# bmds-lab/Crackling

Measured on AMD Instinct MI355X. Metric: guides/sec (whole node) + achieved HBM GB/s, 20bp/<=4mm ISSL scan, higher is better.
Workload: dtype u32

## Files before the change

crackling_amd/csrc/issl_bin.hip:

```cpp
#include <hip/hip_runtime.h>

#include <algorithm>
#include <type_traits>

#include "issl_kernels.hpp"

namespace issl {


__global__ __launch_bounds__(256) void k_pack_scan_stream(ImageView v, uint32_t *__restrict__ scan_out,
                                                          uint64_t *__restrict__ esig_out,
                                                          uint8_t *__restrict__ occ8_out,
                                                          uint32_t *__restrict__ error_flag, uint32_t *__restrict__ seen,
                                                          uint32_t tile_begin, uint32_t tile_end)
{
    for (uint32_t t = tile_begin + blockIdx.x; t < tile_end; t += gridDim.x) {
        uint32_t lo = 0, hi = v.n_buckets;
        while (hi - lo > 1) {
            const uint32_t mid = (lo + hi) >> 1;
            if (v.tile_first[mid] <= t) lo = mid; else hi = mid;
        }
        const uint32_t b = lo;
        const uint32_t slice = b >> v.slice_width;
        const uint64_t start = v.bucket_start[b];
// ... 533 lines not shown
        }
        __syncthreads();
        const uint32_t n_here = total - i0 < THREADS ? total - i0 : THREADS;
        const uint4 *src4 = reinterpret_cast<const uint4 *>(l.stage);
        uint4 *dst4 = reinterpret_cast<uint4 *>(fitems + base.items + i0);
        for (uint32_t q = w; q < n_here * 3u; q += THREADS) dst4[q] = src4[q];
        __syncthreads();
    }
}

template <uint32_t WAYS, uint32_t THREADS>
__device__ __forceinline__ void fine_scatter_guides(const ImageView &v, uint32_t b, const uint32_t *__restrict__ gstart,
                                                    const uint32_t *__restrict__ gfill, const uint32_t *__restrict__ gword,
                                                    const uint32_t *__restrict__ gidx, const uint64_t *__restrict__ gsig,
                                                    const uint32_t *__restrict__ fcount, const uint32_t *__restrict__ fcount0,
                                                    const FineSum *__restrict__ fbase, uint32_t *__restrict__ fword,
                                                    FineMeta *__restrict__ fmeta, FineGuideLds<THREADS> &l)
{
    constexpr uint32_t ways = WAYS;
    const uint32_t w = threadIdx.x, slice = b >> v.slice_width;
    const uint32_t g0 = gstart[b], n = gfill[b];
    const uint32_t base_slots = fbase[b].slots;
    uint32_t c = 0, c1 = 0;
    if (w < 256u) {
        c = fcount[static_cast<uint64_t>(b) * 256u + w];
        c1 = c - fcount0[static_cast<uint64_t>(b) * 256u + w];
    }
    uint32_t i = w, guide = 0, word = 0;
    uint64_t sig = 0;
    if (i < n) { guide = gidx[g0 + i]; word = gword[g0 + i]; sig = gsig[g0 + i]; }
    const uint32_t slots = (c + kGuideGroup - 1u) / kGuideGroup * kGuideGroup;
    const uint32_t slot_at = base_slots + static_cast<uint32_t>(block_exclusive_scan(slots, l.scan, nullptr));
    if (w < 256u) {
        l.slot_of[w] = slot_at;
        l.slot0_of[w] = slot_at + c1;
        l.cursor[w] = 0;
        l.cursor0[w] = 0;
        l.has_cands[w] = c ? 1u : 0u;
        for (uint32_t k2 = c; k2 < slots; ++k2) { fmeta[slot_at + k2] = FineMeta{kNoGuide, 0u, 0ull}; fword[slot_at + k2] = kPadGuideWord; }
    }
    __syncthreads();
    while (i < n) {
        const uint32_t gj = succ_byte(sig, slice, v.slice_width);
        const uint32_t word12 = fine_word(word, slice, v.slice_width);
#pragma unroll
        for (uint32_t way = 0; way < ways; ++way) {
            const uint32_t ww = fine_way(gj, way);
            if (!l.has_cands[ww]) continue;
            const uint32_t slot = way ? l.slot_of[ww] + atomicAdd(&l.cursor[ww], 1u) : l.slot0_of[ww] + atomicAdd(&l.cursor0[ww], 1u);
            fword[slot] = word12 | (fine_class(way) << 24);
            fmeta[slot] = FineMeta{guide, (b << 8) | ww, sig};
        }
        i += THREADS;
        if (i < n) { guide = gidx[g0 + i]; word = gword[g0 + i]; sig = gsig[g0 + i]; }
    }
}

template <uint32_t WAYS, uint32_t THREADS>
__global__ __launch_bounds__(THREADS) void k_fine_scatter(ImageView v, const uint32_t *__restrict__ gstart,
                                                          const uint32_t *__restrict__ gfill, const uint32_t *__restrict__ gword,
                                                          const uint32_t *__restrict__ gidx, const uint64_t *__restrict__ gsig,
                                                          const uint32_t *__restrict__ fcount, const uint32_t *__restrict__ fcount0,
                                                          const FineSum *__restrict__ fbase, const PlanInfo *__restrict__ plan,
                                                          uint32_t *__restrict__ fword, FineMeta *__restrict__ fmeta,
                                                          ScanItem *__restrict__ fitems, uint32_t item_guides, uint32_t tail_shapes)
{
    short_kernel_priority();
    if (!plan->fine) return;
    __shared__ union { FineItemLds<THREADS> items; FineGuideLds<THREADS> guides; } lds;
    const uint32_t nb = v.n_buckets;
    if (blockIdx.x < nb) fine_scatter_items(v, blockIdx.x, fcount, fcount0, fbase, fitems, item_guides, tail_shapes, lds.items);
    else fine_scatter_guides<WAYS, THREADS>(v, blockIdx.x - nb, gstart, gfill, gword, gidx, gsig, fcount, fcount0, fbase, fword, fmeta, lds.guides);
}

__global__ __launch_bounds__(256) void k_fine_ranges(const PlanInfo *__restrict__ plan, const ScanItem *__restrict__ fitems,
                                                     RangeStart *__restrict__ starts)
{
    short_kernel_priority();
    if (!plan->fine) return;
    const uint32_t n_ranges = plan->n_ranges;
    const uint32_t r = blockIdx.x * 4u + (threadIdx.x >> 6);
    if (r <= n_ranges && n_ranges != 0) {
        const RangeStart st = range_start_of<true>(fitems, plan->n_items, plan->total_cost, n_ranges, r);
        if ((threadIdx.x & 63u) == 0u) starts[r] = st;
    }
}

// ... 67 lines not shown
    }
    uint64_t t_units, t_cost, t_cand, t_ref, t_valid;
    uint32_t item_at = static_cast<uint32_t>(block512_exclusive_scan(units, lds, &t_units)) + units_before;
    uint64_t cost_at = block512_exclusive_scan(cost, lds, &t_cost) + cost_before;
    (void)block512_exclusive_scan(cand, lds, &t_cand);
    (void)block512_exclusive_scan(ref, lds, &t_ref);
    const uint32_t slot_at = (static_cast<uint32_t>(block512_exclusive_scan(valid, lds, &t_valid)) + valid_before) * kGuideGroup;
    const uint64_t t_slots = t_valid * kGuideGroup;
    const bool overflow = t_units > ws.cap_fitems || t_slots > ws.cap_fslots;
    if (mine && !overflow && my_s1 > my_s0) {
        const uint32_t way = my_way, s0 = my_s0, s1 = my_s1;
        const uint32_t word12 = fine_word(image_word(sig, sl, v.slice_width, sorted_layout != 0u), sl, v.slice_width);
        const uint32_t ww = fine_way(gj, way);
        const uint32_t c1 = way ? 1u : 0u;
        uint4 *fw = reinterpret_cast<uint4 *>(ws.fword + slot_at);
        fw[0] = make_uint4(word12 | (fine_class(way) << 24), kPadGuideWord, kPadGuideWord, kPadGuideWord);
        fw[1] = make_uint4(kPadGuideWord, kPadGuideWord, kPadGuideWord, kPadGuideWord);
        ws.fmeta[slot_at] = FineMeta{g, (b << 8) | ww, sig};
#pragma unroll
        for (uint32_t k2 = 1; k2 < kGuideGroup; ++k2) ws.fmeta[slot_at + k2] = FineMeta{kNoGuide, 0u, 0ull};
        const GroupUnits gu = group_units(s0, s1, tail_shapes);
        for (uint32_t u = 0; u < gu.units; ++u) {
            const bool full = u < gu.n_full;
            const uint32_t shape = full ? 32u : gu.shape, cap = 64u * shape;
            const uint32_t wstart = gu.s0a + u * kTileCands;
            const uint64_t after = blen - wstart;
            ScanItem it;
            it.bucket = (b << 8) | ww;
            it.g0 = slot_at;
            it.g1 = slot_at + 1u;
            it.n_tiles = 1;
            it.cost0 = cost_at;
            it.tile0 = item_at;
            it.last_cands = after < cap ? static_cast<uint32_t>(after) : cap;
            it.group_abs = tf * 64u + (wstart >> 5);
// ... 74 lines not shown
    hipLaunchKernelGGL(k_guide_scatter, dim3(blocks + range_blocks), dim3(256), 0, stream, d_guides, n, v.slice_width,
                       v.n_slices, (v.srec || v.sid) ? 1u : 0u, nb, ws.gstart, ws.gfill, ws.gword, ws.gidx, ws.gbucket, ws.gsig, blocks, ws.plan, ws.items,
                       ws.range_start);
    if (prune_mode) {
        const uint32_t ways = fine_ways_of(prune_mode);
        const uint32_t tail_shapes = prune_mode == 3 ? 0u : static_cast<uint32_t>(tn.tail_shapes);
        auto launch_fine = [&](auto ways_tag) {
            constexpr uint32_t W = decltype(ways_tag)::value;
            hipLaunchKernelGGL(k_fine_count<W>, dim3(nb), dim3(256), 0, stream, v, ws.gsig, ws.gstart, ws.gfill, ws.fcount,
                               ws.fcount0, ws.fsum, tn.item_guides, tail_shapes);
            hipLaunchKernelGGL(k_fine_plan, dim3(1), dim3(256), 0, stream, ws.fsum, nb, ws.fitems,
                               static_cast<uint32_t>(ws.cap_fitems), static_cast<uint32_t>(ws.cap_fslots), ws.plan, tn.scan_blocks,
                               prune_mode, tn.prune == 1 ? 1u : 0u, ws.sticky, ws.counters);
            if (static_cast<uint64_t>(n) * v.n_slices > 256ull * nb)
                hipLaunchKernelGGL((k_fine_scatter<W, 512u>), dim3(2u * nb), dim3(512), 0, stream, v, ws.gstart, ws.gfill, ws.gword, ws.gidx, ws.gsig,
                                   ws.fcount, ws.fcount0, ws.fsum, ws.plan, ws.fword, ws.fmeta, ws.fitems, tn.item_guides, tail_shapes);
            else
                hipLaunchKernelGGL((k_fine_scatter<W, 256u>), dim3(2u * nb), dim3(256), 0, stream, v, ws.gstart, ws.gfill, ws.gword, ws.gidx, ws.gsig,
                                   ws.fcount, ws.fcount0, ws.fsum, ws.plan, ws.fword, ws.fmeta, ws.fitems, tn.item_guides, tail_shapes);
        };
        if (ways == 1u) launch_fine(std::integral_constant<uint32_t, 1u>{});
        else if (ways == kFineWays) launch_fine(std::integral_constant<uint32_t, kFineWays>{});
        else launch_fine(std::integral_constant<uint32_t, kFineWays2>{});
        hipLaunchKernelGGL(k_fine_ranges, dim3((tn.scan_blocks + 1u + 3u) / 4u), dim3(256), 0, stream, ws.plan, ws.fitems, ws.range_start);
    }
}

}
```

crackling_amd/csrc/issl_device.hpp:

```cpp
#pragma once
#include <cstddef>
#include <cstdint>
#include <string>

#include "issl_host.hpp"

namespace issl {

constexpr uint64_t kImageMagic = 0x314C535349444D41ull;
constexpr uint32_t kImageVersion = 9;
constexpr uint32_t kTileCands = 2048;
constexpr uint32_t kHeaderBytes = 4096;

struct ImageHeader {
    uint64_t magic;
    uint32_t version;
    uint32_t kind;
    uint64_t n_sites, seq_len, n_lines, slice_width, n_slices, n_scores_file;
    uint64_t n_buckets;
    uint64_t n_scores_unique;
    uint64_t n_tiles;
    uint64_t tile_cands;
    uint64_t total_bytes;
    uint64_t off_bucket_start, off_tile_first, off_score_mask, off_score_val, off_sites, off_entries,
// ... 192 lines not shown
#if defined(__HIPCC__)
__host__ __device__
#endif
inline uint64_t slot_pad(uint32_t occ, uint32_t dist) { return static_cast<uint64_t>(occ) | (static_cast<uint64_t>(dist) << 32); }
constexpr uint32_t kFineWays = 13;
constexpr uint32_t kFineWays2 = 67;
constexpr uint32_t kFetchPairs = 8;
constexpr uint32_t kPruneMaxGuides = 1u << 20;
constexpr uint32_t kPruneMaxGuides2 = 1u << 18;
inline uint32_t prune_max_guides(uint32_t prune_mode, uint32_t n_slices)
{
    const uint32_t m = prune_mode == 3 ? kPruneMaxGuides2 : kPruneMaxGuides;
    return n_slices > 10 ? m >> 2 : n_slices > 5 ? m >> 1 : m;
}

struct alignas(16) FineMeta {
    uint32_t guide;
    uint32_t where;
    uint64_t gsig;
};

struct Workspace {
    uint32_t *ng = nullptr;
    uint32_t *gfill = nullptr;
    uint32_t *gstart = nullptr;
    uint32_t *gword = nullptr;
    uint32_t *gidx = nullptr;
    uint32_t *gbucket = nullptr;
    uint64_t *gsig = nullptr;
    ScanItem *items = nullptr;
    uint32_t *fword = nullptr;
    FineMeta *fmeta = nullptr;
    ScanItem *fitems = nullptr;
    uint32_t *fcount = nullptr;
    uint32_t *fcount0 = nullptr;
    FineSum *fsum = nullptr;
    size_t cap_fslots = 0, cap_fitems = 0;
    uint32_t fine_ways = 0;
    PlanInfo *plan = nullptr;
    RangeStart *range_start = nullptr;
    uint64_t *raw = nullptr;
    uint32_t *raw_used = nullptr;
    size_t cap_chunks = 0;
    Counters *counters = nullptr;
    unsigned long long *scan_span = nullptr;
    uint32_t span_slot = 0;
    uint64_t *scan_count = nullptr;
// ... 59 lines not shown
```

crackling_amd/csrc/issl_kernels.hip:

```cpp
#include <hip/hip_runtime.h>

#include "issl_kernels.hpp"

namespace issl {


struct alignas(4 * kGuideGroup) GuideGroup {
    uint32_t w[kGuideGroup];
};


__device__ __forceinline__ uint64_t raw_record(uint32_t gslot, uint32_t tile, uint32_t offset)
{
    return (static_cast<uint64_t>(gslot) << 37) | (static_cast<uint64_t>(tile) << 11) | offset;
}

struct RawWriter {
    uint64_t *chunk;
    uint32_t fill;
    uint32_t left;
    uint32_t reserve;
};

__device__ __forceinline__ void raw_retire(const RawWriter &w, uint32_t lane, const uint64_t *raw, uint32_t *raw_used)
// ... 57 lines not shown
                                                     uint32_t thr, uint32_t keep)
{
    uint32_t m[16];
#pragma unroll
    for (int q = 0; q < 4; ++q) {
        const uint4 lo = gm[q], hi = gm[4 + q];
        asm volatile("" ::: "memory");
        m[4 * q + 0] = (c[4 * q + 0] ^ lo.x) | (c[16 + 4 * q + 0] ^ hi.x);
        m[4 * q + 1] = (c[4 * q + 1] ^ lo.y) | (c[16 + 4 * q + 1] ^ hi.y);
        m[4 * q + 2] = (c[4 * q + 2] ^ lo.z) | (c[16 + 4 * q + 2] ^ hi.z);
        m[4 * q + 3] = (c[4 * q + 3] ^ lo.w) | (c[16 + 4 * q + 3] ^ hi.w);
    }
    return count_near<THR>(m, thr, keep);
}

__device__ __forceinline__ void short_unit_masks(const uint32_t *__restrict__ gword_stream, uint32_t g0, bool wide,
                                                 uint32_t lane, uint4 *lds_masks)
{
    const uint32_t i = lane >> 3, q = lane & 7u;
    uint32_t m[4];
    if (wide) {
        const uint2 gw = *reinterpret_cast<const uint2 *>(gword_stream + g0 + 2u * i);
        const uint32_t a = gw.x >> (4u * q), b = gw.y >> (4u * q);
#pragma unroll
        for (uint32_t r = 0; r < 4; ++r)
            m[r] = ((0u - ((a >> r) & 1u)) & 0xFFFFu) | ((0u - ((b >> r) & 1u)) << 16);
    } else {
        const uint4 gw = *reinterpret_cast<const uint4 *>(gword_stream + g0 + 4u * i);
        const uint32_t t[4] = {gw.x >> (4u * q), gw.y >> (4u * q), gw.z >> (4u * q), gw.w >> (4u * q)};
#pragma unroll
        for (uint32_t r = 0; r < 4; ++r) {
            const uint32_t bits = ((t[0] >> r) & 1u) | (((t[1] >> r) & 1u) << 8) | (((t[2] >> r) & 1u) << 16) | (((t[3] >> r) & 1u) << 24);
            m[r] = bits * 255u;
        }
    }
    lds_masks[i * 8u + q] = make_uint4(m[0], m[1], m[2], m[3]);
}

template <int THR>
__device__ __forceinline__ uint32_t count_near(const uint32_t (&m)[16], uint32_t thr, uint32_t keep)
{
    uint32_t s0, s1, s2, s3, s4, t, u, n0, n1, n2;
    uint32_t k2[8], k4[4], k8a, k8b;
    full_add(m[0], m[1], m[2], s0, k2[0]);
    full_add(m[3], m[4], m[5], s1, k2[1]);
    full_add(m[6], m[7], m[8], s2, k2[2]);
    full_add(m[9], m[10], m[11], s3, k2[3]);
    full_add(m[12], m[13], m[14], s4, k2[4]);
    full_add(s0, s1, s2, t, k2[5]);
// ... 108 lines not shown
        m[4 * q + 3] = (c[4 * q + 3] ^ lo.w) | (c[12 + 4 * q + 3] ^ hi.w);
    }
    const uint32_t f = reinterpret_cast<const uint32_t *>(gm)[24];
    return count_near12<B, true>(m, f, thr, keep, prev);
}

__device__ __forceinline__ uint32_t fine_dup(uint32_t ok, const PrevSlice &prev, uint32_t dup_filter)
{
    const uint32_t prev_mismatch = __builtin_amdgcn_bitop3_b32(prev.a, prev.b, prev.c, 0xFE);
    return ok & (prev_mismatch | ~dup_filter);
}

struct alignas(4) GuideGroupAny {
    uint32_t w[kGuideGroup];
};

constexpr uint32_t fine_order_code(uint32_t slice, uint32_t slice_width)
{
    return fine_order(slice, 0u, slice_width) | (fine_order(slice, 1u, slice_width) << 2) | (fine_order(slice, 2u, slice_width) << 4);
}
constexpr uint32_t kFineOrders = fine_order_code(0u, 8u) | (fine_order_code(1u, 8u) << 6) | (fine_order_code(2u, 8u) << 12) |
                                 (fine_order_code(3u, 8u) << 18) | (fine_order_code(4u, 8u) << 24);
constexpr uint32_t kFineOrderNarrow = fine_order_code(0u, 4u);
static_assert(fine_order_code(0u, 2u) == kFineOrderNarrow && fine_order_code(7u, 4u) == kFineOrderNarrow && (kFineOrders & 63u) == kFineOrderNarrow,
              "narrow slices: one order, that of slice 0 of the 8-bit ones");

struct RecLane {
    uint32_t lo, hi;
};
__device__ __forceinline__ RecLane rec_lane(uint32_t tile, uint32_t off0)
{
    return {(tile << 11) | off0, tile >> 21};
}
__device__ __forceinline__ RecLane rec_lane_at(uint32_t group_abs, uint32_t cand)
{
    const uint64_t at = (static_cast<uint64_t>(group_abs) << 5) + cand;
    return {static_cast<uint32_t>(at), static_cast<uint32_t>(at >> 32)};
}

__device__ __forceinline__ void note_candidates(uint32_t ok, uint32_t gslot, uint32_t w_log, const RecLane &rl,
                                                uint32_t lane, RawWriter &w, uint64_t *raw, uint32_t *raw_used,
                                                uint32_t max_chunks, Counters *counters)
{
    uint64_t who = __ballot(ok != 0u);
    if (who == 0ull) return;
    do {
        const uint32_t n = static_cast<uint32_t>(__builtin_popcountll(who));
        if (__builtin_expect(w.fill + n > kChunkRecs, 0)) {
            raw_retire(w, lane, raw, raw_used);
            raw_acquire(w, raw, max_chunks, counters, lane);
        }
        if (ok != 0u) {
            const uint32_t q = static_cast<uint32_t>(__builtin_ctz(ok));
            ok &= ok - 1u;
            const uint32_t rank = __builtin_amdgcn_mbcnt_hi(static_cast<uint32_t>(who >> 32),
                                                            __builtin_amdgcn_mbcnt_lo(static_cast<uint32_t>(who), 0u));
            const uint32_t lo = rl.lo | (q & ((1u << w_log) - 1u)), hi = rl.hi | ((gslot + (q >> w_log)) << 5);
            w.chunk[w.fill + rank] = (static_cast<uint64_t>(hi) << 32) | lo;
        }
        w.fill += n;
        who = __ballot(ok != 0u);
    } while (__builtin_expect(who != 0ull, 0));
}

template <int THR, bool FINE>
__device__ __forceinline__ void scan_range(const uint32_t *__restrict__ scan_stream, const ScanItem *__restrict__ items,
                                           const PlanInfo *__restrict__ plan, const RangeStart *__restrict__ range_start,
                                           const uint32_t *__restrict__ gword_stream, uint4 *wave_masks,
                                           uint64_t *raw, uint32_t *raw_used, uint32_t max_chunks,
                                           Counters *counters, uint32_t thr, unsigned long long *stamps,
                                           uint64_t *__restrict__ scan_count, uint32_t *next_unit_p, uint32_t *waves_done_p,
                                           unsigned long long *wg_compared_p, unsigned long long t_start,
                                           unsigned long long *span, uint32_t n_tiles, uint32_t slice_bits)
{
    uint32_t &next_unit = *next_unit_p;
    uint32_t &waves_done = *waves_done_p;
    unsigned long long &wg_compared = *wg_compared_p;
    constexpr bool fine = FINE;
    uint32_t units_done = 0;
    unsigned long long plane_wait = 0ull;
    const uint32_t lane = threadIdx.x & 63u;
    const uint32_t wave_id = __builtin_amdgcn_readfirstlane(blockIdx.x * (blockDim.x >> 6) + (threadIdx.x >> 6));
    RawWriter w;
// ... 58 lines not shown
                }
                const int mine0 = static_cast<int>(lane << w_log), width = static_cast<int>(shape);
                const int from = min(max(static_cast<int>(lo) - mine0, 0), width), to = min(max(static_cast<int>(hi) - mine0, 0), width);
                const uint32_t keep = ((1u << to) - (1u << from)) * (wide ? 0x00010001u : 0x01010101u);
                const RecLane rl = rec_lane_at(cur.group_abs, lane << w_log);
                for (uint32_t gb = g_begin; gb < g_end; gb += 8u * per) {
                    __builtin_amdgcn_wave_barrier();
                    short_unit_masks(gword_stream, gb, wide, lane, wave_masks);
                    __builtin_amdgcn_fence(__ATOMIC_RELEASE, "wavefront");
                    __builtin_amdgcn_wave_barrier();
                    const uint32_t passes = (g_end - gb + per - 1u) >> per_log;
                    for (uint32_t i = 0; i < (passes < 8u ? passes : 8u); ++i) {
                        PrevSlice prev;
                        const uint32_t ok = near_plane12_masks<THR>(c, wave_masks + i * 8u, thr, keep, prev);
                        if (__ballot(ok != 0u) != 0ull) {
                            note_candidates(fine_dup(ok, prev, dup_filter), gb + (i << per_log), w_log, rl, lane, w, raw, raw_used, max_chunks, counters);
                            own_chunk = true;
                        }
                    }
                }
                continue;
            }
            const uint32_t at16 = (g0 + lane) << 4;
            const uint32_t off = (at16 & 0x3F0u) + ((at16 & next_tile) << 3);
            uint32_t c[24];
            {
                const uint4 a0 = *reinterpret_cast<const uint4 *>(plane0 - 4096 + off), a1 = *reinterpret_cast<const uint4 *>(plane1 - 4096 + off);
                const uint4 a2 = *reinterpret_cast<const uint4 *>(plane2 - 4096 + off);
                const uint4 b0 = *reinterpret_cast<const uint4 *>(plane0 + off), b1 = *reinterpret_cast<const uint4 *>(plane1 + off);
                const uint4 b2 = *reinterpret_cast<const uint4 *>(plane2 + off);
                c[0] = a0.x; c[1] = a0.y; c[2] = a0.z; c[3] = a0.w; c[4] = a1.x; c[5] = a1.y; c[6] = a1.z; c[7] = a1.w;
                c[8] = a2.x; c[9] = a2.y; c[10] = a2.z; c[11] = a2.w;
                c[12] = b0.x; c[13] = b0.y; c[14] = b0.z; c[15] = b0.w; c[16] = b1.x; c[17] = b1.y; c[18] = b1.z; c[19] = b1.w;
                c[20] = b2.x; c[21] = b2.y; c[22] = b2.z; c[23] = b2.w;
            }
            const int to = min(max(static_cast<int>(hi) - static_cast<int>(lane << 5), 0), 32);
            const uint32_t keep = static_cast<uint32_t>((0xFFFFFFFFull << to) >> 32) & (lane == 0u ? ~0u << lo : ~0u);
            const RecLane rl = rec_lane_at(cur.group_abs, lane << 5);
            if (stamps) {
                const unsigned long long t1 = __builtin_amdgcn_s_memrealtime();
                asm volatile("s_waitcnt vmcnt(0)" ::: "memory");
                plane_wait += __builtin_amdgcn_s_memrealtime() - t1;
            }
            if constexpr (THR < 0) {
                for (uint32_t g = g_begin; g < g_end; g += kGuideGroup) {
                    const GuideGroup gg = *reinterpret_cast<const GuideGroup *>(gword_stream + g);
#pragma unroll
                    for (uint32_t uu = 0; uu < kGuideGroup; ++uu) {
                        if (g + uu >= g_end) break;
                        const uint32_t cls = (gg.w[uu] >> 24) & 3u;
                        if (cls > thr) continue;
                        PrevSlice prev;
                        const uint32_t ok = near_plane12<-1>(c, gg.w[uu], thr - cls, keep, prev);
                        if (__ballot(ok != 0u) != 0ull) {
                            note_candidates(fine_dup(ok, prev, dup_filter), g + uu, 5u, rl, lane, w, raw, raw_used, max_chunks, counters);
                            own_chunk = true;
                        }
                    }
                }
                continue;
            }
            const uint32_t gmid = cur.gmid < g_begin ? g_begin : cur.gmid > g_end ? g_end : cur.gmid;
            if constexpr (THR >= 1) {
                {
                    for (uint32_t g = g_begin; g < gmid; g += kGuideGroup) {
                        const GuideGroupAny gg = *reinterpret_cast<const GuideGroupAny *>(gword_stream + g);
#pragma unroll
                        for (uint32_t uu = 0; uu < kGuideGroup; ++uu) {
                            if (g + uu >= gmid) break;
                            PrevSlice prev;
                            const uint32_t ok = near_plane12<(THR < 1 ? 0 : THR - 1)>(c, gg.w[uu], thr - 1u, keep, prev);
                            if (__ballot(ok != 0u) != 0ull) {
                                note_candidates(fine_dup(ok, prev, dup_filter), g + uu, 5u, rl, lane, w, raw, raw_used, max_chunks, counters);
                                own_chunk = true;
                            }
                        }
                    }
                }
            }
            for (uint32_t g = gmid; g < g_end; g += kGuideGroup) {
                const GuideGroupAny gg = *reinterpret_cast<const GuideGroupAny *>(gword_stream + g);
#pragma unroll
                for (uint32_t uu = 0; uu < kGuideGroup; ++uu) {
                    if (g + uu >= g_end) break;
                    PrevSlice prev;
                    const uint32_t ok = near_plane12<THR>(c, gg.w[uu], thr, keep, prev);
                    if (__ballot(ok != 0u) != 0ull) {
                        note_candidates(fine_dup(ok, prev, dup_filter), g + uu, 5u, rl, lane, w, raw, raw_used, max_chunks, counters);
                        own_chunk = true;
                    }
                }
            }
            continue;
        }

        const uint32_t glane = cur.group_abs + (k << 6) + lane;
        const uint32_t tile = __builtin_amdgcn_readfirstlane(glane >> 6), grp = lane;
        compared += static_cast<unsigned long long>((k + 1u == cur.n_tiles) ? cur.last_cands : kTileCands) * (g_end - g_begin);
        const uint4 *__restrict__ src =
            reinterpret_cast<const uint4 *>(scan_stream + static_cast<uint64_t>(tile) * kTileCands) + grp;
        uint32_t c[kPlanes];
#pragma unroll
        for (int q = 0; q < kPlanes / 4; ++q) {
// ... 6 lines not shown
        const uint32_t keep = (below <= 0 ? ~0u : below >= 32 ? 0u : ~0u << below) &
                              (upto >= 32 ? ~0u : upto <= 0 ? 0u : ~0u >> (32 - upto));
        const RecLane rl = rec_lane(tile, grp * 32u);
        if (stamps) {
            const unsigned long long t1 = __builtin_amdgcn_s_memrealtime();
            asm volatile("s_waitcnt vmcnt(0)" ::: "memory");
            plane_wait += __builtin_amdgcn_s_memrealtime() - t1;
        }
        for (uint32_t g = g_begin; g < g_end; g += kGuideGroup) {
            const GuideGroup gg = *reinterpret_cast<const GuideGroup *>(gword_stream + g);
#pragma unroll
            for (uint32_t uu = 0; uu < kGuideGroup; ++uu) {
                if (g + uu >= g_end) break;
                const uint32_t ok = near_plane<THR>(c, gg.w[uu], thr, keep);
                if (__ballot(ok != 0u) != 0ull) {
                    note_candidates(ok, g + uu, 5u, rl, lane, w, raw, raw_used, max_chunks, counters);
                    own_chunk = true;
                }
            }
        }
    }
    if (own_chunk) {
        raw_retire(w, lane, raw, raw_used);
        if (no_own_chunk && lane == 0) counters->raw_overflow = 1u;
    }
    if (lane == 0) {
        atomicAdd(&wg_compared, compared);
        if (atomicAdd(&waves_done, 1u) == (blockDim.x >> 6) - 1u) {
            scan_count[blockIdx.x] = atomicAdd(&wg_compared, 0ull);
            atomicMax(span + 1, static_cast<unsigned long long>(__builtin_amdgcn_s_memrealtime()));
        }
// ... 2 lines not shown
        stamps[4 * wave_id] = t_start;
        stamps[4 * wave_id + 1] = __builtin_amdgcn_s_memrealtime();
        stamps[4 * wave_id + 2] = (static_cast<unsigned long long>(__builtin_amdgcn_s_getreg((20 << 0) | (0 << 6) | (31 << 11))) << 32) |
                                  __builtin_amdgcn_s_getreg((4 << 0) | (0 << 6) | (31 << 11));
        stamps[4 * wave_id + 3] = units_done | (plane_wait << 32);
    }
}

template <int THR>
__global__ __launch_bounds__(1024, 8) void k_scan(const uint32_t *__restrict__ scan_stream,
                                                  const ScanItem *__restrict__ items_full,
                                                  const ScanItem *__restrict__ items_fine,
                                                  const PlanInfo *__restrict__ plan,
                                                  const RangeStart *__restrict__ range_start,
                                                  const uint32_t *__restrict__ gword_full,
                                                  const uint32_t *__restrict__ gword_fine, uint64_t *raw,
                                                  uint32_t *raw_used, uint32_t max_chunks, Counters *counters, uint32_t thr,
                                                  unsigned long long *stamps, uint64_t *__restrict__ scan_count,
                                                  unsigned long long *span, uint32_t n_tiles, uint32_t slice_bits)
{
    __shared__ uint32_t next_unit;
    __shared__ uint32_t waves_done;
    __shared__ unsigned long long wg_compared;
    __shared__ uint4 tail_masks[16][64];
    const unsigned long long t_start = __builtin_amdgcn_s_memrealtime();
    if (threadIdx.x == 0) { next_unit = 0; waves_done = 0; wg_compared = 0ull; }
    __syncthreads();
    if (blockIdx.x >= plan->n_ranges) {
        if (threadIdx.x == 0) scan_count[blockIdx.x] = 0ull;
        return;
    }
    if (threadIdx.x == 0) atomicMin(span, t_start);
    if (plan->fine != 0u)
        scan_range<THR, true>(scan_stream, items_fine, plan, range_start, gword_fine, tail_masks[threadIdx.x >> 6], raw, raw_used, max_chunks, counters, thr, stamps,
                              scan_count, &next_unit, &waves_done, &wg_compared, t_start, span, n_tiles, slice_bits);
    else
        scan_range<THR, false>(scan_stream, items_full, plan, range_start, gword_full, tail_masks[threadIdx.x >> 6], raw, raw_used, max_chunks, counters, thr, stamps,
                               scan_count, &next_unit, &waves_done, &wg_compared, t_start, span, n_tiles, slice_bits);
}

template <int THR>
static void launch_scan_thr(const ImageView &v, const Workspace &ws, const Tuning &tn, uint32_t thr, uint32_t prune_mode,
                            hipStream_t stream)
{
    hipLaunchKernelGGL(k_scan<THR>, dim3(tn.scan_blocks), dim3(tn.scan_threads), 0, stream, v.scan, ws.items,
                       prune_mode ? ws.fitems : ws.items, ws.plan, ws.range_start, ws.gword, prune_mode ? ws.fword : ws.gword,
                       ws.raw, ws.raw_used, static_cast<uint32_t>(ws.cap_chunks), ws.counters, thr, ws.stamps, ws.scan_count,
                       ws.scan_span + 2u * ws.span_slot, v.n_tiles, v.slice_width);
}

void launch_scan(const ImageView &v, const Workspace &ws, const Tuning &tn, const uint64_t *d_guides, uint32_t n,
                 int max_dist, uint32_t prune_mode, void *stream_)
{
    (void)n;
    (void)d_guides;
    hipStream_t stream = static_cast<hipStream_t>(stream_);
    if (max_dist < 0) {
        (void)hipMemsetAsync(ws.scan_count, 0, 8ull * tn.scan_blocks, stream);
        return;
    }
    const uint32_t thr = max_dist > 31 ? 31u : static_cast<uint32_t>(max_dist);
// ... 10 lines not shown
```

crackling_amd/csrc/issl_pipeline.cpp:

```cpp
#include <algorithm>
#include <cstdio>
#include <cstring>
#include <vector>

#include "issl_index.hpp"

namespace issl {

int supported_geometry(const Geometry &g)
{
    if (g.seq_len == 20 && (g.slice_width == 8 || g.slice_width == 4 || g.slice_width == 2) && g.n_slices * g.slice_width == 40) return ISSL_OK;
    set_error("unsupported index geometry: the gfx950 scan kernels implement 20 bp sequences in slices of 8, 4 or 2 bits "
              "(got seq_len=" + std::to_string(g.seq_len) + " slice_width=" +
              std::to_string(g.slice_width) + " slices=" + std::to_string(g.n_slices) + ")");
    return ISSL_E_UNSUPPORTED;
}

int select_device(int device)
{
    int count = 0;
    hipError_t e = hipGetDeviceCount(&count);
    if (e != hipSuccess || count <= 0) {
        set_error("no HIP device available: the ISSL scorer has no CPU fallback");
        return ISSL_E_DEVICE;
    }
    if (device < 0 || device >= count) {
        set_error("device " + std::to_string(device) + " out of range (" + std::to_string(count) + " visible)");
        return ISSL_E_ARG;
    }
    HIP_TRY(hipSetDevice(device));
    return ISSL_OK;
}

static void free_workspace(Workspace &w)
{
    void *ptrs[] = {w.ng, w.gfill, w.gstart, w.gword, w.gidx, w.gbucket, w.gsig, w.items, w.plan, w.range_start, w.counters, w.scan_count, w.scan_span, w.sticky, w.stamps, w.gcur_big, w.gcur_big2, w.terms, w.sorted, w.gcount,
                    w.goff, w.blocksum, w.d_guides, w.d_mit, w.d_cfd, w.d_kept, w.d_hitrec, w.pay, w.rank, w.fword, w.fmeta,
                    w.fitems, w.fcount, w.fcount0, w.fsum, w.slots};
    for (void *p : ptrs)
        if (p) (void)hipFree(p);
    if (w.raw) (void)hipFree(w.raw);
    if (w.raw_used) (void)hipFree(w.raw_used);
    if (w.h_stage) (void)hipHostFree(w.h_stage);
    w = Workspace{};
}

void release_lanes(issl_index *ix)
{
    for (Lane *lp : {&ix->lane, &ix->lane2}) {
        Lane &lane = *lp;
        if (lane.ready) {
            (void)hipStreamSynchronize(lane.stream);
// ... 120 lines not shown
        }
        w.cap_guides = cap;
        w.cap_gslots = slots;
        w.cap_items = items;
    }
    if (ix->hdr.off_sub_start && (grew || fine_ways > w.fine_ways)) {
        const size_t cap = w.cap_guides;
        const uint32_t ways = std::max(fine_ways, w.fine_ways);
        const size_t m = std::min<size_t>(cap, prune_max_guides(ways > kFineWays ? 3u : 2u, ix->hdr.n_slices));
        const size_t places = m * ix->hdr.n_slices * ways;
        const size_t groups = std::min<size_t>(nb * 256, places);
        const size_t fslots = places + kGuideGroup * groups;
        const size_t tiles_per_group = static_cast<size_t>(ix->hdr.n_sites * ix->hdr.n_slices / (static_cast<uint64_t>(nb) * 256ull * kTileCands)) + 4;
        const size_t fitems = std::max<size_t>(tn.fine_items ? tn.fine_items : tiles_per_group * (groups + places / 64) + 2, w.cap_fitems);
        if ((rc = dev_alloc(w.fword, fslots + 64))) return rc;
        if ((rc = dev_alloc(w.fmeta, fslots))) return rc;
        if ((rc = dev_alloc(w.fitems, fitems + 1))) return rc;
        if ((rc = dev_alloc(w.fcount, nb * 256))) return rc;
        if ((rc = dev_alloc(w.fcount0, nb * 256))) return rc;
        if ((rc = dev_alloc(w.fsum, nb))) return rc;
        w.cap_fslots = fslots;
        w.cap_fitems = fitems;
        w.fine_ways = ways;
    }

    if (w.cap_chunks == 0) {
        const size_t want = tn.raw_chunks ? tn.raw_chunks : std::max<size_t>(size_t(scan_waves(tn)) * 6, n);
        if ((rc = ensure_raw_capacity(w, want))) return rc;
    }
    if (!ix->have_events) {
        for (auto &e : ix->ring) HIP_TRY(hipEventCreate(&e));
// ... 552 lines not shown
```

crackling_amd/csrc/issl_verify.hip:

```cpp
#include <hip/hip_runtime.h>

#include <algorithm>

#include "issl_kernels.hpp"

namespace issl {

__global__ __launch_bounds__(kChunkRecs, 8) void k_verify(ImageView v, Workspace ws, const uint64_t *__restrict__ guides,
                                                       ScoreParams p)
{
    short_kernel_priority();
    const int max_dist = p.max_dist;
    const bool calc_mit = p.method == ISSL_METHOD_MIT || p.method == ISSL_METHOD_AND || p.method == ISSL_METHOD_OR ||
                          p.method == ISSL_METHOD_AVG;
    const bool calc_cfd = p.method == ISSL_METHOD_CFD || p.method == ISSL_METHOD_AND || p.method == ISSL_METHOD_OR ||
                          p.method == ISSL_METHOD_AVG;
    const uint32_t prune_mode = ws.plan->fine;
    uint32_t n_chunks = ws.counters->raw_chunks;
    if (blockIdx.x == 0 && threadIdx.x == 0) {
        if (ws.counters->raw_overflow) atomicOr(&ws.sticky[0], 1u);
        atomicMax(&ws.sticky[1], n_chunks);
        if (ws.plan->error) atomicOr(&ws.sticky[2], ws.plan->error);
    }
    if (n_chunks > ws.cap_chunks) n_chunks = static_cast<uint32_t>(ws.cap_chunks);
// ... 4 lines not shown
        const uint64_t rec_any = recs[t < kChunkRecs ? t : 0u];
        const uint32_t used = ws.raw_used[chunk];
        const bool in_use = t < used && t < kChunkRecs;
        const uint64_t rec = in_use ? rec_any : 0ull;
        uint64_t key = kDeadKey;
        double mit_term = 0.0, cfd_term = 0.0;
        uint64_t hit_gsig = 0, hit_ot = 0;
        uint32_t hit_occ = 0;
        const uint32_t offset = static_cast<uint32_t>(rec) & (kTileCands - 1u);
        const uint32_t tile = static_cast<uint32_t>(rec >> 11) & 0x3FFFFFFu;
        const uint32_t gslot = static_cast<uint32_t>(rec >> 37);
        const bool by_id = v.srec || v.sid;
        StreamRec sr_early{};
        if (in_use && v.srec) sr_early = v.srec[static_cast<uint64_t>(tile) * kTileCands + offset];
        else if (in_use && v.sid) sr_early.id = v.sid[static_cast<uint64_t>(tile) * kTileCands + offset];
        uint32_t guide = kNoGuide, where = 0;
        uint64_t gsig = 0;
        if (in_use) {
            if (prune_mode) { const FineMeta m = ws.fmeta[gslot]; guide = m.guide; where = m.where; gsig = m.gsig; }
            else { guide = ws.gidx[gslot]; where = ws.gbucket[gslot]; }
        }
        if (guide != kNoGuide) {
            const uint32_t bucket = prune_mode ? where >> 8 : where;
            const uint32_t slice = bucket >> v.slice_width;
            uint64_t start = 0, pos = 0;
            bool mine = true;
            if (!by_id) {
                start = v.bucket_start[bucket];
                pos = static_cast<uint64_t>(tile - v.tile_first[bucket]) * kTileCands + offset;
                mine = pos < v.bucket_start[bucket + 1] - start;
            }
            if (mine) {
                if (!prune_mode) gsig = guides[guide];
                StreamRec sr = sr_early;
                if (v.sid) sr.sig = v.sites[sr.id];
                const uint64_t ot = by_id    ? sr.sig & kSigMask
                                    : v.esig ? v.esig[start + pos]
                                    : v.occ8 ? candidate_signature(v, bucket, tile, offset)
                                             : v.sites[v.entries[start + pos] & 0xFFFFFFFFull];
// ... 68 lines not shown
            if (rank < kMidHits) {
                int dist;
                score_terms(v, hit_gsig, hit_ot, hit_occ, calc_mit, calc_cfd, mit_term, cfd_term, dist);
                reinterpret_cast<double2 *>(ws.pay)[slot] = make_double2(mit_term, cfd_term);
            }
        }
        if (!in_use) continue;
        if (!ws.lean_tail) recs[t] = key;
    }
}

void launch_verify(const ImageView &v, const Workspace &ws, const uint64_t *d_guides, uint32_t n, const ScoreParams &p, void *stream)
{
    if (p.max_dist < 0) return;
    const uint32_t grid = n < 256u ? std::max<uint32_t>(2048u, 64u * n) : kTailGrid;
    hipLaunchKernelGGL(k_verify, dim3(std::min(grid, kTailGrid)), dim3(kChunkRecs), 0, static_cast<hipStream_t>(stream), v, ws, d_guides, p);
}

}
```

Before: 45.68 million.

## Interleave fine slot words with packed guide/slice ids, drop FineMeta array

After: 47.69 million, median of 6. 1.04x the previous value.

```diff
diff --git a/crackling_amd/csrc/issl_bin.hip b/crackling_amd/csrc/issl_bin.hip
--- a/crackling_amd/csrc/issl_bin.hip
+++ b/crackling_amd/csrc/issl_bin.hip
@@ -571,8 +571,8 @@
                                                     const uint32_t *__restrict__ gfill, const uint32_t *__restrict__ gword,
                                                     const uint32_t *__restrict__ gidx, const uint64_t *__restrict__ gsig,
                                                     const uint32_t *__restrict__ fcount, const uint32_t *__restrict__ fcount0,
-                                                    const FineSum *__restrict__ fbase, uint32_t *__restrict__ fword,
-                                                    FineMeta *__restrict__ fmeta, FineGuideLds<THREADS> &l)
+                                                    const FineSum *__restrict__ fbase, FineSlot *__restrict__ fword,
+                                                    FineGuideLds<THREADS> &l)
 {
     constexpr uint32_t ways = WAYS;
     const uint32_t w = threadIdx.x, slice = b >> v.slice_width;
@@ -594,19 +594,18 @@
         l.cursor[w] = 0;
         l.cursor0[w] = 0;
         l.has_cands[w] = c ? 1u : 0u;
-        for (uint32_t k2 = c; k2 < slots; ++k2) { fmeta[slot_at + k2] = FineMeta{kNoGuide, 0u, 0ull}; fword[slot_at + k2] = kPadGuideWord; }
+        for (uint32_t k2 = c; k2 < slots; ++k2) fword[slot_at + k2] = FineSlot{kPadGuideWord, kPadSlotId};
     }
     __syncthreads();
     while (i < n) {
         const uint32_t gj = succ_byte(sig, slice, v.slice_width);
-        const uint32_t word12 = fine_word(word, slice, v.slice_width);
+        const uint32_t word12 = fine_word(word, slice, v.slice_width), id = slot_id(slice, guide);
 #pragma unroll
         for (uint32_t way = 0; way < ways; ++way) {
             const uint32_t ww = fine_way(gj, way);
             if (!l.has_cands[ww]) continue;
             const uint32_t slot = way ? l.slot_of[ww] + atomicAdd(&l.cursor[ww], 1u) : l.slot0_of[ww] + atomicAdd(&l.cursor0[ww], 1u);
-            fword[slot] = word12 | (fine_class(way) << 24);
-            fmeta[slot] = FineMeta{guide, (b << 8) | ww, sig};
+            fword[slot] = FineSlot{word12 | (fine_class(way) << 24), id};
         }
         i += THREADS;
         if (i < n) { guide = gidx[g0 + i]; word = gword[g0 + i]; sig = gsig[g0 + i]; }
@@ -619,7 +618,7 @@
                                                           const uint32_t *__restrict__ gidx, const uint64_t *__restrict__ gsig,
                                                           const uint32_t *__restrict__ fcount, const uint32_t *__restrict__ fcount0,
                                                           const FineSum *__restrict__ fbase, const PlanInfo *__restrict__ plan,
-                                                          uint32_t *__restrict__ fword, FineMeta *__restrict__ fmeta,
+                                                          FineSlot *__restrict__ fword,
                                                           ScanItem *__restrict__ fitems, uint32_t item_guides, uint32_t tail_shapes)
 {
     short_kernel_priority();
@@ -627,7 +626,7 @@
     __shared__ union { FineItemLds<THREADS> items; FineGuideLds<THREADS> guides; } lds;
     const uint32_t nb = v.n_buckets;
     if (blockIdx.x < nb) fine_scatter_items(v, blockIdx.x, fcount, fcount0, fbase, fitems, item_guides, tail_shapes, lds.items);
-    else fine_scatter_guides<WAYS, THREADS>(v, blockIdx.x - nb, gstart, gfill, gword, gidx, gsig, fcount, fcount0, fbase, fword, fmeta, lds.guides);
+    else fine_scatter_guides<WAYS, THREADS>(v, blockIdx.x - nb, gstart, gfill, gword, gidx, gsig, fcount, fcount0, fbase, fword, lds.guides);
 }
 
 __global__ __launch_bounds__(256) void k_fine_ranges(const PlanInfo *__restrict__ plan, const ScanItem *__restrict__ fitems,
@@ -725,11 +724,9 @@
         const uint32_t ww = fine_way(gj, way);
         const uint32_t c1 = way ? 1u : 0u;
         uint4 *fw = reinterpret_cast<uint4 *>(ws.fword + slot_at);
-        fw[0] = make_uint4(word12 | (fine_class(way) << 24), kPadGuideWord, kPadGuideWord, kPadGuideWord);
-        fw[1] = make_uint4(kPadGuideWord, kPadGuideWord, kPadGuideWord, kPadGuideWord);
-        ws.fmeta[slot_at] = FineMeta{g, (b << 8) | ww, sig};
+        fw[0] = make_uint4(word12 | (fine_class(way) << 24), slot_id(sl, g), kPadGuideWord, kPadSlotId);
 #pragma unroll
-        for (uint32_t k2 = 1; k2 < kGuideGroup; ++k2) ws.fmeta[slot_at + k2] = FineMeta{kNoGuide, 0u, 0ull};
+        for (uint32_t k2 = 1; k2 < kGuideGroup / 2u; ++k2) fw[k2] = make_uint4(kPadGuideWord, kPadSlotId, kPadGuideWord, kPadSlotId);
         const GroupUnits gu = group_units(s0, s1, tail_shapes);
         for (uint32_t u = 0; u < gu.units; ++u) {
             const bool full = u < gu.n_full;
@@ -834,10 +831,10 @@
                                prune_mode, tn.prune == 1 ? 1u : 0u, ws.sticky, ws.counters);
             if (static_cast<uint64_t>(n) * v.n_slices > 256ull * nb)
                 hipLaunchKernelGGL((k_fine_scatter<W, 512u>), dim3(2u * nb), dim3(512), 0, stream, v, ws.gstart, ws.gfill, ws.gword, ws.gidx, ws.gsig,
-                                   ws.fcount, ws.fcount0, ws.fsum, ws.plan, ws.fword, ws.fmeta, ws.fitems, tn.item_guides, tail_shapes);
+                                   ws.fcount, ws.fcount0, ws.fsum, ws.plan, ws.fword, ws.fitems, tn.item_guides, tail_shapes);
             else
                 hipLaunchKernelGGL((k_fine_scatter<W, 256u>), dim3(2u * nb), dim3(256), 0, stream, v, ws.gstart, ws.gfill, ws.gword, ws.gidx, ws.gsig,
-                                   ws.fcount, ws.fcount0, ws.fsum, ws.plan, ws.fword, ws.fmeta, ws.fitems, tn.item_guides, tail_shapes);
+                                   ws.fcount, ws.fcount0, ws.fsum, ws.plan, ws.fword, ws.fitems, tn.item_guides, tail_shapes);
         };
         if (ways == 1u) launch_fine(std::integral_constant<uint32_t, 1u>{});
         else if (ways == kFineWays) launch_fine(std::integral_constant<uint32_t, kFineWays>{});
diff --git a/crackling_amd/csrc/issl_device.hpp b/crackling_amd/csrc/issl_device.hpp
--- a/crackling_amd/csrc/issl_device.hpp
+++ b/crackling_amd/csrc/issl_device.hpp
@@ -230,10 +230,28 @@
     return n_slices > 10 ? m >> 2 : n_slices > 5 ? m >> 1 : m;
 }
 
-struct alignas(16) FineMeta {
-    uint32_t guide;
-    uint32_t where;
-    uint64_t gsig;
+constexpr uint32_t kSlotIdBits = 27, kSlotGuideBits = 22;
+constexpr uint32_t kPadSlotId = (1u << kSlotIdBits) - 1u;
+#if defined(__HIPCC__)
+__host__ __device__
+#endif
+inline uint32_t slot_id(uint32_t slice, uint32_t guide) { return (slice << kSlotGuideBits) | guide; }
+#if defined(__HIPCC__)
+__host__ __device__
+#endif
+inline void slot_id_unpack(uint32_t id, uint32_t &slice, uint32_t &guide)
+{
+    slice = id >> kSlotGuideBits;
+    guide = id & ((1u << kSlotGuideBits) - 1u);
+}
+static_assert(kPruneMaxGuides <= (1u << kSlotGuideBits), "a pruned launch's guides fit the id's guide field");
+static_assert(kMaxSlices <= (1u << (kSlotIdBits - kSlotGuideBits)), "an index's slices fit the id's slice field");
+static_assert(((kMaxSlices - 1u) << kSlotGuideBits | (kPruneMaxGuides - 1u)) < kPadSlotId, "no slot's id is the padding id");
+static_assert(kSlotIdBits + 26u + 11u == 64u, "raw record: slot id, tile, offset in tile");
+
+struct alignas(8) FineSlot {
+    uint32_t word;
+    uint32_t id;
 };
 
 struct Workspace {
@@ -245,8 +263,7 @@
     uint32_t *gbucket = nullptr;
     uint64_t *gsig = nullptr;
     ScanItem *items = nullptr;
-    uint32_t *fword = nullptr;
-    FineMeta *fmeta = nullptr;
+    FineSlot *fword = nullptr;
     ScanItem *fitems = nullptr;
     uint32_t *fcount = nullptr;
     uint32_t *fcount0 = nullptr;
diff --git a/crackling_amd/csrc/issl_kernels.hip b/crackling_amd/csrc/issl_kernels.hip
--- a/crackling_amd/csrc/issl_kernels.hip
+++ b/crackling_amd/csrc/issl_kernels.hip
@@ -1,4 +1,6 @@
 #include <hip/hip_runtime.h>
+
+#include <type_traits>
 
 #include "issl_kernels.hpp"
 
@@ -95,25 +97,30 @@
     return count_near<THR>(m, thr, keep);
 }
 
-__device__ __forceinline__ void short_unit_masks(const uint32_t *__restrict__ gword_stream, uint32_t g0, bool wide,
+constexpr uint32_t kPassIds = 28;
+typedef uint32_t SlotPair __attribute__((ext_vector_type(4)));
+__device__ __forceinline__ void short_unit_masks(const FineSlot *__restrict__ slots, uint32_t g0, bool wide,
                                                  uint32_t lane, uint4 *lds_masks)
 {
     const uint32_t i = lane >> 3, q = lane & 7u;
     uint32_t m[4];
     if (wide) {
-        const uint2 gw = *reinterpret_cast<const uint2 *>(gword_stream + g0 + 2u * i);
-        const uint32_t a = gw.x >> (4u * q), b = gw.y >> (4u * q);
+        const SlotPair gw = *reinterpret_cast<const SlotPair *>(slots + g0 + 2u * i);
+        const uint32_t a = gw.x >> (4u * q), b = gw.z >> (4u * q);
 #pragma unroll
         for (uint32_t r = 0; r < 4; ++r)
             m[r] = ((0u - ((a >> r) & 1u)) & 0xFFFFu) | ((0u - ((b >> r) & 1u)) << 16);
+        if (q == 7u) { m[0] = gw.y; m[1] = gw.w; }
     } else {
-        const uint4 gw = *reinterpret_cast<const uint4 *>(gword_stream + g0 + 4u * i);
-        const uint32_t t[4] = {gw.x >> (4u * q), gw.y >> (4u * q), gw.z >> (4u * q), gw.w >> (4u * q)};
+        const SlotPair *src = reinterpret_cast<const SlotPair *>(slots + g0 + 4u * i);
+        const SlotPair ga = src[0], gb = src[1];
+        const uint32_t t[4] = {ga.x >> (4u * q), ga.z >> (4u * q), gb.x >> (4u * q), gb.z >> (4u * q)};
 #pragma unroll
         for (uint32_t r = 0; r < 4; ++r) {
             const uint32_t bits = ((t[0] >> r) & 1u) | (((t[1] >> r) & 1u) << 8) | (((t[2] >> r) & 1u) << 16) | (((t[3] >> r) & 1u) << 24);
             m[r] = bits * 255u;
         }
+        if (q == 7u) { m[0] = ga.y; m[1] = ga.w; m[2] = gb.y; m[3] = gb.w; }
     }
     lds_masks[i * 8u + q] = make_uint4(m[0], m[1], m[2], m[3]);
 }
@@ -252,6 +259,9 @@
 struct alignas(4) GuideGroupAny {
     uint32_t w[kGuideGroup];
 };
+struct alignas(8) FineSlotGroup {
+    FineSlot s[kGuideGroup];
+};
 
 constexpr uint32_t fine_order_code(uint32_t slice, uint32_t slice_width)
 {
@@ -276,7 +286,7 @@
     return {static_cast<uint32_t>(at), static_cast<uint32_t>(at >> 32)};
 }
 
-__device__ __forceinline__ void note_candidates(uint32_t ok, uint32_t gslot, uint32_t w_log, const RecLane &rl,
+__device__ __forceinline__ void note_candidates(uint32_t ok, uint32_t gslot, const uint32_t *pass_ids, uint32_t w_log, const RecLane &rl,
                                                 uint32_t lane, RawWriter &w, uint64_t *raw, uint32_t *raw_used,
                                                 uint32_t max_chunks, Counters *counters)
 {
@@ -293,7 +303,8 @@
             ok &= ok - 1u;
             const uint32_t rank = __builtin_amdgcn_mbcnt_hi(static_cast<uint32_t>(who >> 32),
                                                             __builtin_amdgcn_mbcnt_lo(static_cast<uint32_t>(who), 0u));
-            const uint32_t lo = rl.lo | (q & ((1u << w_log) - 1u)), hi = rl.hi | ((gslot + (q >> w_log)) << 5);
+            const uint32_t slot = pass_ids ? pass_ids[q >> w_log] : gslot + (q >> w_log);
+            const uint32_t lo = rl.lo | (q & ((1u << w_log) - 1u)), hi = rl.hi | (slot << 5);
             w.chunk[w.fill + rank] = (static_cast<uint64_t>(hi) << 32) | lo;
         }
         w.fill += n;
@@ -304,7 +315,7 @@
 template <int THR, bool FINE>
 __device__ __forceinline__ void scan_range(const uint32_t *__restrict__ scan_stream, const ScanItem *__restrict__ items,
                                            const PlanInfo *__restrict__ plan, const RangeStart *__restrict__ range_start,
-                                           const uint32_t *__restrict__ gword_stream, uint4 *wave_masks,
+                                           const std::conditional_t<FINE, FineSlot, uint32_t> *__restrict__ gword_stream, uint4 *wave_masks,
                                            uint64_t *raw, uint32_t *raw_used, uint32_t max_chunks,
                                            Counters *counters, uint32_t thr, unsigned long long *stamps,
                                            uint64_t *__restrict__ scan_count, uint32_t *next_unit_p, uint32_t *waves_done_p,
@@ -393,7 +404,8 @@
                         PrevSlice prev;
                         const uint32_t ok = near_plane12_masks<THR>(c, wave_masks + i * 8u, thr, keep, prev);
                         if (__ballot(ok != 0u) != 0ull) {
-                            note_candidates(fine_dup(ok, prev, dup_filter), gb + (i << per_log), w_log, rl, lane, w, raw, raw_used, max_chunks, counters);
+                            note_candidates(fine_dup(ok, prev, dup_filter), 0u, reinterpret_cast<const uint32_t *>(wave_masks + i * 8u) + kPassIds, w_log, rl, lane, w, raw,
+                                            raw_used, max_chunks, counters);
                             own_chunk = true;
                         }
                     }
@@ -423,16 +435,16 @@
             }
             if constexpr (THR < 0) {
                 for (uint32_t g = g_begin; g < g_end; g += kGuideGroup) {
-                    const GuideGroup gg = *reinterpret_cast<const GuideGroup *>(gword_stream + g);
+                    const FineSlotGroup gg = *reinterpret_cast<const FineSlotGroup *>(gword_stream + g);
 #pragma unroll
                     for (uint32_t uu = 0; uu < kGuideGroup; ++uu) {
                         if (g + uu >= g_end) break;
-                        const uint32_t cls = (gg.w[uu] >> 24) & 3u;
+                        const uint32_t cls = (gg.s[uu].word >> 24) & 3u;
                         if (cls > thr) continue;
                         PrevSlice prev;
-                        const uint32_t ok = near_plane12<-1>(c, gg.w[uu], thr - cls, keep, prev);
+                        const uint32_t ok = near_plane12<-1>(c, gg.s[uu].word, thr - cls, keep, prev);
                         if (__ballot(ok != 0u) != 0ull) {
-                            note_candidates(fine_dup(ok, prev, dup_filter), g + uu, 5u, rl, lane, w, raw, raw_used, max_chunks, counters);
+                            note_candidates(fine_dup(ok, prev, dup_filter), gg.s[uu].id, nullptr, 5u, rl, lane, w, raw, raw_used, max_chunks, counters);
                             own_chunk = true;
                         }
                     }
@@ -443,14 +455,14 @@
             if constexpr (THR >= 1) {
                 {
                     for (uint32_t g = g_begin; g < gmid; g += kGuideGroup) {
-                        const GuideGroupAny gg = *reinterpret_cast<const GuideGroupAny *>(gword_stream + g);
+                        const FineSlotGroup gg = *reinterpret_cast<const FineSlotGroup *>(gword_stream + g);
 #pragma unroll
                         for (uint32_t uu = 0; uu < kGuideGroup; ++uu) {
                             if (g + uu >= gmid) break;
                             PrevSlice prev;
-                            const uint32_t ok = near_plane12<(THR < 1 ? 0 : THR - 1)>(c, gg.w[uu], thr - 1u, keep, prev);
+                            const uint32_t ok = near_plane12<(THR < 1 ? 0 : THR - 1)>(c, gg.s[uu].word, thr - 1u, keep, prev);
                             if (__ballot(ok != 0u) != 0ull) {
-                                note_candidates(fine_dup(ok, prev, dup_filter), g + uu, 5u, rl, lane, w, raw, raw_used, max_chunks, counters);
+                                note_candidates(fine_dup(ok, prev, dup_filter), gg.s[uu].id, nullptr, 5u, rl, lane, w, raw, raw_used, max_chunks, counters);
                                 own_chunk = true;
                             }
                         }
@@ -458,14 +470,14 @@
                 }
             }
             for (uint32_t g = gmid; g < g_end; g += kGuideGroup) {
-                const GuideGroupAny gg = *reinterpret_cast<const GuideGroupAny *>(gword_stream + g);
+                const FineSlotGroup gg = *reinterpret_cast<const FineSlotGroup *>(gword_stream + g);
 #pragma unroll
                 for (uint32_t uu = 0; uu < kGuideGroup; ++uu) {
                     if (g + uu >= g_end) break;
                     PrevSlice prev;
-                    const uint32_t ok = near_plane12<THR>(c, gg.w[uu], thr, keep, prev);
+                    const uint32_t ok = near_plane12<THR>(c, gg.s[uu].word, thr, keep, prev);
                     if (__ballot(ok != 0u) != 0ull) {
-                        note_candidates(fine_dup(ok, prev, dup_filter), g + uu, 5u, rl, lane, w, raw, raw_used, max_chunks, counters);
+                        note_candidates(fine_dup(ok, prev, dup_filter), gg.s[uu].id, nullptr, 5u, rl, lane, w, raw, raw_used, max_chunks, counters);
                         own_chunk = true;
                     }
                 }
@@ -502,7 +514,7 @@
                 if (g + uu >= g_end) break;
                 const uint32_t ok = near_plane<THR>(c, gg.w[uu], thr, keep);
                 if (__ballot(ok != 0u) != 0ull) {
-                    note_candidates(ok, g + uu, 5u, rl, lane, w, raw, raw_used, max_chunks, counters);
+                    note_candidates(ok, g + uu, nullptr, 5u, rl, lane, w, raw, raw_used, max_chunks, counters);
                     own_chunk = true;
                 }
             }
@@ -535,7 +547,7 @@
                                                   const PlanInfo *__restrict__ plan,
                                                   const RangeStart *__restrict__ range_start,
                                                   const uint32_t *__restrict__ gword_full,
-                                                  const uint32_t *__restrict__ gword_fine, uint64_t *raw,
+                                                  const FineSlot *__restrict__ gword_fine, uint64_t *raw,
                                                   uint32_t *raw_used, uint32_t max_chunks, Counters *counters, uint32_t thr,
                                                   unsigned long long *stamps, uint64_t *__restrict__ scan_count,
                                                   unsigned long long *span, uint32_t n_tiles, uint32_t slice_bits)
@@ -565,7 +577,7 @@
                             hipStream_t stream)
 {
     hipLaunchKernelGGL(k_scan<THR>, dim3(tn.scan_blocks), dim3(tn.scan_threads), 0, stream, v.scan, ws.items,
-                       prune_mode ? ws.fitems : ws.items, ws.plan, ws.range_start, ws.gword, prune_mode ? ws.fword : ws.gword,
+                       prune_mode ? ws.fitems : ws.items, ws.plan, ws.range_start, ws.gword, ws.fword,
                        ws.raw, ws.raw_used, static_cast<uint32_t>(ws.cap_chunks), ws.counters, thr, ws.stamps, ws.scan_count,
                        ws.scan_span + 2u * ws.span_slot, v.n_tiles, v.slice_width);
 }
diff --git a/crackling_amd/csrc/issl_pipeline.cpp b/crackling_amd/csrc/issl_pipeline.cpp
--- a/crackling_amd/csrc/issl_pipeline.cpp
+++ b/crackling_amd/csrc/issl_pipeline.cpp
@@ -35,7 +35,7 @@
 static void free_workspace(Workspace &w)
 {
     void *ptrs[] = {w.ng, w.gfill, w.gstart, w.gword, w.gidx, w.gbucket, w.gsig, w.items, w.plan, w.range_start, w.counters, w.scan_count, w.scan_span, w.sticky, w.stamps, w.gcur_big, w.gcur_big2, w.terms, w.sorted, w.gcount,
-                    w.goff, w.blocksum, w.d_guides, w.d_mit, w.d_cfd, w.d_kept, w.d_hitrec, w.pay, w.rank, w.fword, w.fmeta,
+                    w.goff, w.blocksum, w.d_guides, w.d_mit, w.d_cfd, w.d_kept, w.d_hitrec, w.pay, w.rank, w.fword,
                     w.fitems, w.fcount, w.fcount0, w.fsum, w.slots};
     for (void *p : ptrs)
         if (p) (void)hipFree(p);
@@ -186,7 +186,6 @@
         const size_t tiles_per_group = static_cast<size_t>(ix->hdr.n_sites * ix->hdr.n_slices / (static_cast<uint64_t>(nb) * 256ull * kTileCands)) + 4;
         const size_t fitems = std::max<size_t>(tn.fine_items ? tn.fine_items : tiles_per_group * (groups + places / 64) + 2, w.cap_fitems);
         if ((rc = dev_alloc(w.fword, fslots + 64))) return rc;
-        if ((rc = dev_alloc(w.fmeta, fslots))) return rc;
         if ((rc = dev_alloc(w.fitems, fitems + 1))) return rc;
         if ((rc = dev_alloc(w.fcount, nb * 256))) return rc;
         if ((rc = dev_alloc(w.fcount0, nb * 256))) return rc;
diff --git a/crackling_amd/csrc/issl_verify.hip b/crackling_amd/csrc/issl_verify.hip
--- a/crackling_amd/csrc/issl_verify.hip
+++ b/crackling_amd/csrc/issl_verify.hip
@@ -7,7 +7,7 @@
 namespace issl {
 
 __global__ __launch_bounds__(kChunkRecs, 8) void k_verify(ImageView v, Workspace ws, const uint64_t *__restrict__ guides,
-                                                       ScoreParams p)
+                                                       uint32_t n, ScoreParams p)
 {
     short_kernel_priority();
     const int max_dist = p.max_dist;
@@ -42,15 +42,23 @@
         StreamRec sr_early{};
         if (in_use && v.srec) sr_early = v.srec[static_cast<uint64_t>(tile) * kTileCands + offset];
         else if (in_use && v.sid) sr_early.id = v.sid[static_cast<uint64_t>(tile) * kTileCands + offset];
-        uint32_t guide = kNoGuide, where = 0;
+        uint32_t guide = kNoGuide, bucket = 0, slice = 0;
         uint64_t gsig = 0;
         if (in_use) {
-            if (prune_mode) { const FineMeta m = ws.fmeta[gslot]; guide = m.guide; where = m.where; gsig = m.gsig; }
-            else { guide = ws.gidx[gslot]; where = ws.gbucket[gslot]; }
+            if (prune_mode) {
+                if (gslot != kPadSlotId) slot_id_unpack(gslot, slice, guide);
+                if (guide >= n || slice >= v.n_slices) guide = kNoGuide;
+                else {
+                    gsig = guides[guide];
+                    bucket = (slice << v.slice_width) + (static_cast<uint32_t>(gsig >> (v.slice_width * slice)) & static_cast<uint32_t>(low));
+                }
+            } else {
+                guide = ws.gidx[gslot];
+                bucket = ws.gbucket[gslot];
+                slice = bucket >> v.slice_width;
+            }
         }
         if (guide != kNoGuide) {
-            const uint32_t bucket = prune_mode ? where >> 8 : where;
-            const uint32_t slice = bucket >> v.slice_width;
             uint64_t start = 0, pos = 0;
             bool mine = true;
             if (!by_id) {
@@ -149,7 +157,7 @@
 {
     if (p.max_dist < 0) return;
     const uint32_t grid = n < 256u ? std::max<uint32_t>(2048u, 64u * n) : kTailGrid;
-    hipLaunchKernelGGL(k_verify, dim3(std::min(grid, kTailGrid)), dim3(kChunkRecs), 0, static_cast<hipStream_t>(stream), v, ws, d_guides, p);
+    hipLaunchKernelGGL(k_verify, dim3(std::min(grid, kTailGrid)), dim3(kChunkRecs), 0, static_cast<hipStream_t>(stream), v, ws, d_guides, n, p);
 }
 
 }
```
